# Xiuyu-Li/q-diffusion

Hardware: AMD Instinct MI355X
Metric: denoising images/sec (whole node), SD-v1.4 W4A8 512x512 50-step PLMS (higher is better)
Workload: dtype int8xint4->int32 (fp32 residual stream); 1 GPU; sd UNet eval batch 16 per GPU, 51 evals per image batch, W4A8 sm_abit=16 split, hip-graph=on, cross-attention K/V of the run's context prepared once per image batch (2.93 ms, charged as /51 per step); images_per_gpu=8, global_batch=8, context_prepared=True, parallelism=batch-sharded x1, quant-state broadcast 0 B

## Files before the change

### include/qdiff_hip.h

```cpp
#ifndef QDIFF_HIP_H
#define QDIFF_HIP_H

#include <stdint.h>

#ifdef __cplusplus
extern "C" {
#endif

#define QD_ABI_VERSION 20

enum { QD_F32 = 0, QD_F16 = 1, QD_BF16 = 2 };
enum { QD_EPI_LINEAR = 0, QD_EPI_GEGLU_I8 = 1, QD_EPI_HEADS_I8 = 2, QD_EPI_HEADS_T_I8 = 3, QD_EPI_GEGLU_H16 = 4  };

int         qd_abi_version(void);
const char* qd_last_error(void);
int         qd_device_ok(void);

int qd_box_probe(int kind, int blocks, int iters, long long* ticks, int* sink, void* stream);

int qd_make_qparams(const float* delta, const float* zero_point, float* out4, void* stream);

int qd_quantize_act(const void* x, int x_dtype, int64_t B, int64_t C, int64_t S,
                    int64_t sb, int64_t sc, int64_t ss,
                    int c0, int clen, int clen_pad,
// ... 32 lines not shown
    int32_t        out_dtype;
    int32_t        nseg;
    int32_t        w_tiled;
    int32_t        epilogue;
    qd_conv_seg    seg[2];
    const float*   oq_params;
    int32_t        oq_min, oq_max, oq_off, _pad2;
    void*          splitk_ws;
    int64_t        splitk_ws_bytes;
    int32_t        hd_H, hd_d, hd_T, hd_Tpad, hd_dpad;
    float          oq_prescale;
    int32_t*       hd_sum;
    float*         gn_part;
    int64_t        gn_ld;
    int32_t        upsample2x;
    int32_t        _pad3;
} qd_conv_desc;

int qd_conv2d_i8(const qd_conv_desc* d, void* stream);

void qd_conv_config(int kgroups);

int qd_conv2d_i8_group(const qd_conv_desc* const* descs, int n, void* stream);

int64_t qd_conv2d_i8_splitk_ws_bytes(const qd_conv_desc* d);

int qd_pack_weights_t4(const float* w, const float* alpha, const float* delta, const float* zp,
                       int Cout, int Cin_total, int taps, int c0, int clen, int clen_pad, int n_levels,
                       uint8_t* wt, int kstep0, int ntiles, int32_t* wsum, void* stream);

int qd_pack_weights_t8(const float* w, const float* alpha, const float* delta, const float* zp,
                       int Cout, int Cin_total, int taps, int c0, int clen, int clen_pad, int n_levels,
                       uint8_t* wt, int kstep0, int ntiles, int32_t* wsum, void* stream);

int qd_conv2d_i8_acc(const qd_conv_desc* d, int32_t* iout, void* stream);

// ... 112 lines not shown
```

### q-diffusion_amd/csrc/common.h

```cpp
#pragma once
#include <hip/hip_runtime.h>
#include <hip/hip_fp16.h>
#include <hip/hip_bf16.h>
#include <stdint.h>
#include <type_traits>
#include "../../include/qdiff_hip.h"

typedef int   v4i  __attribute__((ext_vector_type(4)));
typedef int   v16i __attribute__((ext_vector_type(16)));
typedef float v4f  __attribute__((ext_vector_type(4)));

void qd_set_error(const char* fmt, ...);

#define QD_REQUIRE(cond, ...)                 \
    do {                                      \
        if (!(cond)) {                        \
            qd_set_error(__VA_ARGS__);        \
            return 1;                         \
        }                                     \
    } while (0)

#define QD_LAUNCH_CHECK(name)                                                       \
    do {                                                                            \
        hipError_t e__ = hipGetLastError();                                         \
// ... 75 lines not shown
template <typename T>
__device__ __forceinline__ void qd_ld4(const T* p, bool vec, float (&v)[4]) {
    if (vec) {
        if constexpr (sizeof(T) == 4) {
            const float4 f = *reinterpret_cast<const float4*>(p);
            v[0] = f.x; v[1] = f.y; v[2] = f.z; v[3] = f.w;
        } else {
            const uint2 u = *reinterpret_cast<const uint2*>(p);
            const __half2 a = *reinterpret_cast<const __half2*>(&u.x), b = *reinterpret_cast<const __half2*>(&u.y);
            v[0] = __low2float(a); v[1] = __high2float(a); v[2] = __low2float(b); v[3] = __high2float(b);
        }
    } else {
#pragma unroll
        for (int j = 0; j < 4; ++j) v[j] = qd_ld(p + j);
    }
}

__device__ __forceinline__ float qd_erff(float a) {
    const float t = __builtin_fabsf(a), s = a * a;
    float r = __builtin_fmaf(-1.72853470e-5f, t, 3.83197126e-4f);
    const float u = __builtin_fmaf(-3.88396438e-3f, t, 2.42546219e-2f);
    r = __builtin_fmaf(r, s, u);
    r = __builtin_fmaf(r, t, -1.06777877e-1f);
    r = __builtin_fmaf(r, t, -6.34846687e-1f);
    r = __builtin_fmaf(r, t, -1.28717512e-1f);
    r = __builtin_fmaf(r, t, -t);
    const float big = __builtin_copysignf(1.0f - __builtin_amdgcn_exp2f(r * 1.4426950408889634f), a);
    float q = -5.96761703e-4f;
    q = __builtin_fmaf(q, s, 4.99119423e-3f);
    q = __builtin_fmaf(q, s, -2.67681349e-2f);
// ... 110 lines not shown
```

### q-diffusion_amd/csrc/igemm_dma.hip

```cpp
#include "common.h"
#include <type_traits>

typedef __attribute__((address_space(3))) void* qd_lds_ptr;

namespace {

__device__ __attribute__((aligned(16))) const int qd_zero16[4] = {0, 0, 0, 0};

struct SegD {
    int c0, clen, kstep0, nsteps_tap;
    const float*  scale;
    const int*    zc;
    const int*    zw;
    const int*    zfill;
    const int8_t* fill16;
};

struct ConvD {
    const int8_t*  x;
    const uint8_t* wt;
    void*          out;
    int32_t*       iout;
    const float*   bias;
    const float*   rowbias;
// ... 1122 lines not shown
        vals[j] = code;
    }
    unsigned w0 = 0, w1 = 0;
#pragma unroll
    for (int b = 0; b < 4; ++b) {
        w0 |= (unsigned)((vals[b] & 15) | ((vals[4 + b] & 15) << 4)) << (8 * b);
        w1 |= (unsigned)((vals[8 + b] & 15) | ((vals[12 + b] & 15) << 4)) << (8 * b);
    }
    const long kstep = kstep0 + (long)t * nsteps_tap + cs;
    uint2 pk = {w0, w1};
    *reinterpret_cast<uint2*>(wt + (kstep * ntiles + jt) * 1024 + (kh4 * 32 + nn) * 8) = pk;
    if (wsum && sum != 0) atomicAdd(&wsum[n], sum);
}

template <typename TO>
__global__ __launch_bounds__(256) void splitk_finalize_kernel(const int32_t* __restrict__ part, int nsplit, long MN, int Cout, int HoWo,
                                                              const float* __restrict__ scale, const int* __restrict__ zc,
                                                              const int* __restrict__ zw, const int* __restrict__ zfill,
                                                              const float* __restrict__ bias, const float* __restrict__ rowbias, long ldrb,
                                                              const TO* __restrict__ residual, long ldr, TO* __restrict__ out, long ldo) {
    const long e = (long)blockIdx.x * 256 + threadIdx.x;
    if (e >= MN) return;
    const long m = e / Cout;
    const int  n = (int)(e - m * Cout);
    int I = 0;
    for (int s = 0; s < nsplit; ++s) I += part[(long)s * MN + e];
    const int kz = zfill ? zfill[1] : 0;
    I = I - (zc ? zc[n] : 0) + (zw ? zw[n] : 0) * kz;
    float v = __builtin_fmaf((float)I, scale[n], bias ? bias[n] : 0.f);
    if (rowbias) v += rowbias[(m / HoWo) * ldrb + n];
    if constexpr (std::is_same<TO, float>::value) {
        if (residual) v += residual[m * ldr + n];
        out[m * ldo + n] = v;
    } else {
        if (residual) v += __half2float(residual[m * ldr + n]);
        out[m * ldo + n] = __float2half(v);
    }
}

__global__ __launch_bounds__(256) void pack_t8_kernel(const float* __restrict__ w, const float* __restrict__ alpha,
                                                      const float* __restrict__ delta, const float* __restrict__ zp,
                                                      int Cout, int Cin_total, int taps, int c0, int clen,
                                                      int n_levels, uint8_t* __restrict__ wt, int kstep0, int ntiles,
                                                      int nsteps_tap, int32_t* __restrict__ wsum) {
    long gid = (long)blockIdx.x * 256 + threadIdx.x;
    const long total = (long)taps * nsteps_tap * ntiles * 128;
    if (gid >= total) return;
    const int nn = (int)(gid & 31);
    const int kh4 = (int)((gid >> 5) & 3);
    long rest = gid >> 7;
    const int jt = (int)(rest % ntiles);
// ... 80 lines not shown
        QD_CASE(false, O_F32) QD_CASE(false, O_F16)
    } else {
        QD_CASE(false, O_F32)
        QD_CASE(false, O_F16)
        if constexpr (MT == 1 && WM == 4) { QD_CASE(false, O_I32) QD_CASE(true, O_F32) QD_CASE(true, O_F16) QD_CASE(false, O_PART) }
        if constexpr ((WB == 4 && WM == 4) || (WB == 8 && MT == 1 && NT == 4)) { QD_CASE(false, O_HROWS) QD_CASE(false, O_HTR) }
        if constexpr (NT == 4 && WB == 4 && WM == 4) { QD_CASE(false, O_GEGLU) }
    }
#undef QD_CASE
    qd_set_error("qd_conv2d_%s: unsupported variant split=%d out=%d tile %dx%d", WB >= 16 ? "bf16" : "i8", (int)split, out, BM, BN);
    return 1;
}

int nt_for(int N) { return N % 160 == 0 ? 5 : (N % 224 == 0 ? 7 : (N > 64 ? 4 : 2)); }

int choose_splitk(const qd_conv_desc* d, int* it_per) {
    *it_per = 0;
    if (d->nseg != 1 || d->epilogue != QD_EPI_LINEAR) return 1;
    const long M = (long)d->B * d->Ho * d->Wo;
    const int  N = d->Cout, bn = 32 * (d->wbits == 8 ? (N > 64 ? 4 : 2) : nt_for(N));
    const long blocks0 = ((M + 127) / 128) * ((N + bn - 1) / bn);
    const int  total = d->kh * d->kw * ((d->seg[0].clen + 63) / 64);
    if (blocks0 > 256) return 1;
    const long mn = M * N;
    const int min_steps = mn <= (1L << 18) ? 2 : (mn <= (3L << 19) ? 4 : 16);
    static const long target = getenv("QD_SPLITK_TARGET") ? atol(getenv("QD_SPLITK_TARGET")) : 256;
    long S = target / blocks0;
    if (S > total / min_steps) S = total / min_steps;
    if (S > 32) S = 32;
    if (S < 2) return 1;
    *it_per = (int)((total + S - 1) / S);
    return (total + *it_per - 1) / *it_per;
}

int run(const qd_conv_desc* d, int32_t* iout, void* stream) {
    QD_REQUIRE(d != nullptr, "qd_conv2d_i8: null descriptor");
    QD_REQUIRE(d->x && d->w && (d->out || iout), "qd_conv2d_i8: null tensor pointer");
// ... 52 lines not shown
        QD_REQUIRE(d->hd_Tpad % 32 == 0 && d->hd_Tpad >= d->hd_T && d->hd_dpad >= d->hd_d, "qd_conv2d_i8: heads epilogue: bad padded dims");
        QD_REQUIRE(qd_aligned(d->out, 16) && (d->epilogue != QD_EPI_HEADS_T_I8 || d->hd_sum), "qd_conv2d_i8: heads epilogue: out unaligned or hd_sum missing");
        QD_REQUIRE(!d->rowbias && (!d->residual || (d->epilogue == QD_EPI_HEADS_I8 && d->ldr % 4 == 0 && qd_aligned(d->residual, 4 * esz))),
                   "qd_conv2d_i8: heads epilogue takes no rowbias; a residual (fp32 or fp16 as out_dtype says, 4-element aligned rows) only with QD_EPI_HEADS_I8");
        k.res_f16 = d->out_dtype == QD_F16 ? 1 : 0;
        k.vec = (d->epilogue == QD_EPI_HEADS_I8 && d->hd_d % 8 == 0 && d->hd_dpad % 8 == 0 && d->Cout % 8 == 0 && qd_aligned(d->out, 8) &&
                 (!d->residual || (d->ldr % 8 == 0 && qd_aligned(d->residual, 16)))) ? 2 : 1;
        k.oq = d->oq_params; k.oqmin = (float)d->oq_min; k.oqmax = (float)d->oq_max; k.oqoff = d->oq_off;
        k.hdH = d->hd_H; k.hdd = d->hd_d; k.hdT = d->hd_T; k.hdTpad = d->hd_Tpad; k.hddpad = d->hd_dpad;
        k.oqpre = d->oq_prescale; k.hdsum = d->hd_sum;
        QD_REQUIRE(d->Cout < 65536, "qd_conv2d_i8: heads epilogue: Cout must be < 65536");
        k.hdrcp = (unsigned)((0x100000000ULL + (unsigned)d->hd_d - 1) / (unsigned)d->hd_d);
    }
    if (d->gn_part) {
        QD_REQUIRE(!iout && !heads && !geglu, "qd_conv2d_i8: gn_part needs the plain fp32 / fp16 epilogue");
        QD_REQUIRE((d->Ho * d->Wo) % 128 == 0, "qd_conv2d_i8: gn_part needs Ho*Wo %% 128 == 0 (a 128-row chunk stays inside one sample)");
        k.gnpart = d->gn_part;
        k.gn_nchunk = d->Ho * d->Wo / 128;
        QD_REQUIRE(d->gn_ld == 0 || d->gn_ld >= d->Cout, "qd_conv2d_i8: gn_ld must be 0 or >= Cout");
        k.gn_ld = d->gn_ld ? (long)d->gn_ld : (long)d->Cout;
    }
    const bool mt2_ok = !heads || d->hd_T % 256 == 0;
    if (geglu) {
        QD_REQUIRE(!iout && d->nseg == 1 && d->oq_params && d->Cout % 64 == 0, "qd_conv2d_i8: GEGLU epilogue needs one segment, oq_params and Cout %% 64 == 0");
        QD_REQUIRE(d->oq_max - d->oq_off <= 127 && d->oq_min - d->oq_off >= -128, "qd_conv2d_i8: GEGLU output grid does not fit int8");
        QD_REQUIRE(d->ldo % 16 == 0 && qd_aligned(d->out, 16), "qd_conv2d_i8: GEGLU output rows must be 16-byte aligned");
        k.oq = d->oq_params; k.oqmin = (float)d->oq_min; k.oqmax = (float)d->oq_max; k.oqoff = d->oq_off;
    }
    QD_REQUIRE(!(iout && split), "qd_conv2d_i8_acc: single segment only");
    hipStream_t st = reinterpret_cast<hipStream_t>(stream);
    const int N = d->Cout;
    const long M = k.M;
    int rc;
    auto blocks = [&](int bm, int bn) { return ((M + bm - 1) / bm) * ((N + bn - 1) / bn); };
    int it_per = 0;
    const int nsplit = (iout || !d->splitk_ws || d->gn_part) ? 1 : choose_splitk(d, &it_per);
    if (nsplit >= 2 && d->splitk_ws_bytes >= (int64_t)nsplit * M * N * 4) {
        QD_REQUIRE(qd_aligned(d->splitk_ws, 16), "qd_conv2d_i8: splitk_ws must be 16-byte aligned");
        k.iout = reinterpret_cast<int32_t*>(d->splitk_ws);
        k.it_per = it_per;
        k.vec = N % 4 == 0;
        if (w8) rc = N > 64 ? dispatch<1, 4, 4, 1, 8>(k, false, O_PART, st, nsplit) : dispatch<1, 2, 4, 1, 8>(k, false, O_PART, st, nsplit);
        else switch (nt_for(N)) {
            case 5:  rc = dispatch<1, 5, 4, 1>(k, false, O_PART, st, nsplit); break;
            case 7:  rc = dispatch<1, 7, 4, 1>(k, false, O_PART, st, nsplit); break;
            case 4:  rc = dispatch<1, 4, 4, 1>(k, false, O_PART, st, nsplit); break;
            default: rc = dispatch<1, 2, 4, 1>(k, false, O_PART, st, nsplit); break;
        }
        if (rc || g_capture) return rc;
        const SegD& sg = k.seg[0];
        const long MN = M * N;
        dim3 grid((unsigned)((MN + 255) / 256)), block(256);
        if (d->out_dtype == QD_F16)
            hipLaunchKernelGGL(splitk_finalize_kernel<__half>, grid, block, 0, st, k.iout, nsplit, MN, N, d->Ho * d->Wo, sg.scale, sg.zc, sg.zw,
                               sg.zfill, k.bias, k.rowbias, k.ldrb, (const __half*)k.residual, k.ldr, (__half*)k.out, k.ldo);
        else
            hipLaunchKernelGGL(splitk_finalize_kernel<float>, grid, block, 0, st, k.iout, nsplit, MN, N, d->Ho * d->Wo, sg.scale, sg.zc, sg.zw,
                               sg.zfill, k.bias, k.rowbias, k.ldrb, (const float*)k.residual, k.ldr, (float*)k.out, k.ldo);
        QD_LAUNCH_CHECK("qd_conv2d_i8 (split-K)");
        return 0;
    }
    static const int wide_mink = getenv("QD_WIDE_MINK") ? atoi(getenv("QD_WIDE_MINK")) : 1280;
    static const int wide_minblk = getenv("QD_WIDE_MINBLK") ? atoi(getenv("QD_WIDE_MINBLK")) : 200;
    const long Ktot = (long)k.taps * d->seg[0].clen;
    const bool linear_out = out == O_F32 || out == O_F16;
    auto want_mt2 = [&](int bn) {
        if (split || !mt2_ok || out == O_I32) return false;
        if (g_capture) return false;
// ... 177 lines not shown
        if (ok) {
            QD_LAUNCH_CHECK("qd_conv2d_i8_group");
            return 0;
        }
    }
    for (int i = 0; i < n; ++i) {
        const int rc = run(descs[i], nullptr, stream);
        if (rc) return rc;
    }
    return 0;
}

extern "C" void qd_conv_config(int kgroups) {
    if (kgroups >= 0) kgroups_knob() = kgroups ? 1 : 0;
}
extern "C" int qd_conv2d_i8_group(const qd_conv_desc* const* descs, int n, void* stream) { return run_group(descs, n, stream); }
extern "C" int qd_conv2d_i8(const qd_conv_desc* d, void* stream) { return run(d, nullptr, stream); }
extern "C" int qd_conv2d_i8_acc(const qd_conv_desc* d, int32_t* iout, void* stream) {
    if (!iout) { qd_set_error("qd_conv2d_i8_acc: null iout"); return 1; }
    return run(d, iout, stream);
}

extern "C" int qd_pack_weights_t4(const float* w, const float* alpha, const float* delta, const float* zp, int Cout,
                                  int Cin_total, int taps, int c0, int clen, int clen_pad, int n_levels, uint8_t* wt,
                                  int kstep0, int ntiles, int32_t* wsum, void* stream) {
    QD_REQUIRE(w && delta && zp && wt, "qd_pack_weights_t4: null pointer");
    QD_REQUIRE(Cout > 0 && taps > 0 && clen > 0 && c0 >= 0 && c0 + clen <= Cin_total, "qd_pack_weights_t4: bad shape");
    QD_REQUIRE(clen_pad % 16 == 0 && clen_pad >= clen, "qd_pack_weights_t4: clen_pad must be a multiple of 16");
    QD_REQUIRE(n_levels >= 2 && n_levels <= 16, "qd_pack_weights_t4: n_levels %d does not fit a nibble", n_levels);
    QD_REQUIRE(ntiles == (Cout + 31) / 32 && qd_aligned(wt, 16), "qd_pack_weights_t4: bad tile layout");
// ... 584 lines not shown
```

### q-diffusion_amd/csrc/norm_quant.hip

```cpp
#include "common.h"

namespace {

static inline __host__ __device__ int gn_rows(long S) { return S > 256 ? 32 : 8; }

template <typename T>
__global__ __launch_bounds__(256) void gn_partial_kernel(const T* __restrict__ x, long S, int C, long ldx,
                                                         float* __restrict__ part, int nchunk, int vec) {
    const int chunk = blockIdx.x;
    const long b = blockIdx.y;
    const int rows = gn_rows(S);
    const long r0 = (long)chunk * rows;
    const long r1 = (r0 + rows < S) ? r0 + rows : S;
    for (int c4 = threadIdx.x; c4 < C / 4; c4 += 256) {
        float s[4] = {0, 0, 0, 0}, q[4] = {0, 0, 0, 0};
        const T* p = x + (b * S + r0) * ldx + c4 * 4;
#pragma unroll 4
        for (long r = r0; r < r1; ++r, p += ldx) {
            float v[4];
            qd_ld4(p, vec != 0, v);
#pragma unroll
            for (int j = 0; j < 4; ++j) {
                s[j] += v[j];
                q[j] += v[j] * v[j];
            }
        }
        float* dst = part + (((b * nchunk + chunk) * (long)C) + c4 * 4) * 2;
        *reinterpret_cast<float4*>(dst)     = make_float4(s[0], q[0], s[1], q[1]);
        *reinterpret_cast<float4*>(dst + 4) = make_float4(s[2], q[2], s[3], q[3]);
    }
}

__global__ __launch_bounds__(256) void gn_partial_h8_kernel(const __half* __restrict__ x, long S, int C, long ldx,
                                                            float* __restrict__ part, int nchunk) {
    const int chunk = blockIdx.x;
    const long b = blockIdx.y;
    const int rows = gn_rows(S);
    const long r0 = (long)chunk * rows;
    const long r1 = (r0 + rows < S) ? r0 + rows : S;
    for (int c8 = threadIdx.x; c8 < C / 8; c8 += 256) {
        float s[8] = {0, 0, 0, 0, 0, 0, 0, 0}, q[8] = {0, 0, 0, 0, 0, 0, 0, 0};
        const __half* p = x + (b * S + r0) * ldx + c8 * 8;
#pragma unroll 4
        for (long r = r0; r < r1; ++r, p += ldx) {
            float v[8];
            qd_ld8h(p, v);
#pragma unroll
            for (int j = 0; j < 8; ++j) {
                s[j] += v[j];
                q[j] += v[j] * v[j];
            }
        }
        float* dst = part + (((b * nchunk + chunk) * (long)C) + c8 * 8) * 2;
#pragma unroll
        for (int j = 0; j < 4; ++j) *reinterpret_cast<float4*>(dst + 4 * j) = make_float4(s[2 * j], q[2 * j], s[2 * j + 1], q[2 * j + 1]);
    }
}

template <int NT>
__global__ __launch_bounds__(NT) void gn_finalize_kernel(const float* __restrict__ part, int nchunk, long ldp, long S, int C,
                                                         int groups, float eps, const float* __restrict__ gamma,
                                                         const float* __restrict__ beta, float* __restrict__ ab) {
    static_assert(NT == 64 || NT == 256, "one wave, or four whose results are added in wave order");
    const int g = blockIdx.x;
    const long b = blockIdx.y;
    const int cpg = C / groups;
// ... 1026 lines not shown
```

### q-diffusion_amd/qdiff/engine.py

```python
import math

import os

import torch

from . import hip
from .hip import Grid, pad16, pad32

SIMULATE = False


class simulation:

    def __enter__(self):
        global SIMULATE
        self.prev, SIMULATE = SIMULATE, True
        return self

    def __exit__(self, *exc):
        global SIMULATE
        SIMULATE = self.prev
        return False


# ... 283 lines not shown

    def __init__(self, slot, i):
        self.slot, self.i = slot, i

    def rows(self, M, C, device):
        return self.slot.rows(self.i, M, C, device)

    def part(self, B, nchunk, C, device):
        return self.slot.part(self.i, B, nchunk, C, device)


def upsample_fold_ok(plan, H, W):
    return bool(plan.pack.tiled and plan.kh * plan.kw > 1 and plan.stride == 1 and H % 2 == 0 and W % 2 == 0)


def conv_forward(plan, xq, B, H, W, Ho=None, Wo=None, out=None, rowbias=None, residual=None, acc_out=None,
                 out_dtype=None, pad_tl=None, splitk=None, gn_stats=False, slot=None, upsample2x=False):
    if Ho is None:
        Ho, Wo = conv_out_hw(H, W, plan)
    M = B * Ho * Wo
    if out_dtype is None:
        out_dtype = out.dtype if out is not None else stream_dtype()
    if residual is not None and acc_out is None and residual.dtype != out_dtype:
        residual = residual.to(out_dtype)
    if out is None and acc_out is None:
        if slot is not None and out_dtype == stream_dtype():
            out = slot.rows(M, plan.Cout, xq.device)
        if out is None:
            slot = None
            out = torch.empty((M, plan.Cout), dtype=out_dtype, device=xq.device)
    else:
        slot = None
    pad = plan.pad if pad_tl is None else pad_tl
    call = hip.ConvCall(x=xq, w=plan.pack.wq, out=out, bias=plan.bias, rowbias=rowbias,
                        residual=residual, ldx=plan.ldx, ldk=plan.pack.ldk,
                        ldo=(out.stride(0) if out is not None else 0),
                        ldr=(residual.stride(0) if residual is not None else 0),
                        ld_rowbias=(rowbias.stride(0) if rowbias is not None else 0),
                        B=B, H=H, W=W, Ho=Ho, Wo=Wo, Cout=plan.Cout, kh=plan.kh, kw=plan.kw, stride=plan.stride,
                        pad_t=pad, pad_l=pad, wbits=plan.pack.wbits, w_tiled=plan.pack.tiled, segs=plan.segs,
                        splitk=splitk, upsample2x=upsample2x)
    part = None
    if (gn_stats and acc_out is None and plan.pack.tiled and out.dtype in (torch.float32, torch.float16) and (Ho * Wo) % 128 == 0
            and out.stride(1) == 1 and (splitk is False or hip.splitk_ws_bytes(call) == 0)):
        if slot is not None:
            part = slot.part(B, Ho * Wo // 128, plan.Cout, xq.device)
        if part is None:
            part = torch.empty((B, Ho * Wo // 128, plan.Cout, 2), dtype=torch.float32, device=xq.device)
        call.gn_part = part
    hip.conv2d_i8(call, acc_out=acc_out)
    if part is not None:
        out.qd_gn_part = part
    return out if acc_out is None else acc_out


def conv_forward_geglu(plan, xq, M, next_plan):
    if not plan.pack.tiled or plan.pack.wbits != 4 or plan.pack.row_perm is None or len(plan.segs) != 1 or len(next_plan.segs) != 1:
        raise hip.HipEngineError("fused GEGLU epilogue needs a tile-ordered int4 projection packed with geglu_row_perm")
    out = torch.empty((M, next_plan.ldx), dtype=torch.int8, device=xq.device)
    call = hip.ConvCall(x=xq, w=plan.pack.wq, out=out, bias=plan.bias, ldx=plan.ldx, ldk=plan.pack.ldk, ldo=next_plan.ldx,
                        B=1, H=1, W=M, Ho=1, Wo=M, Cout=plan.Cout, kh=1, kw=1, stride=1, pad_t=0, pad_l=0,
                        wbits=plan.pack.wbits, w_tiled=True, segs=plan.segs, epilogue=hip.EPI_GEGLU_I8,
                        oq_params=next_plan.qparams[0], oq_grid=next_plan.grids[0])
    hip.conv2d_i8(call)
# ... 314 lines not shown


_ws_cache = {}


def _workspace(nbytes, device):
    key = (device, torch.cuda.current_stream().cuda_stream if device.type == "cuda" else 0)
    buf = _ws_cache.get(key)
    if buf is None or buf.numel() < nbytes:
        buf = torch.empty(max(nbytes, 1 << 20), dtype=torch.uint8, device=device)
        _ws_cache[key] = buf
    return buf


def _part_view(part, B, S, C):
    if part is None or S % 128 != 0 or part.dim() != 4 or part.shape[2] != C or part.shape[0] * part.shape[1] * 128 != B * S:
        return None
    if tuple(part.shape[:2]) == (B, S // 128):
        return part
    try:
        return part.view(B, S // 128, C, 2)
    except RuntimeError:
        return None


def raw_quant_segs(plan, C):
    segs, pos = [], 0
    for sg, d, grid, qp in zip(plan.pack.segs, plan.segs, plan.grids, plan.qparams):
        if sg["clen"] % 16 or sg["c0w"] % 16 or d["c0"] % 16 or sg["c0w"] != pos:
            return None
        segs.append(dict(c0=sg["c0w"], clen=sg["clen"], oc0=d["c0"], qparams=qp, grid=grid))
        pos += sg["clen"]
    return segs if pos == C and 1 <= len(segs) <= 2 else None


def groupnorm_silu_quant(x_rows, B, S, C, gn, silu, plan=None, want_float=False, part=None, raw_plan=None, mod=None):
# ... 285 lines not shown
```

### q-diffusion_amd/qdiff/hip.py

```python
import ctypes
import os

import torch

_HERE = os.path.dirname(os.path.abspath(__file__))
LIB_PATH = os.environ.get("QDIFF_HIP_LIB") or os.path.join(os.path.dirname(_HERE), "lib", "libqdiff_hip.so")

F32, F16, BF16 = 0, 1, 2
_DT = {torch.float32: F32, torch.float16: F16}


class HipEngineError(RuntimeError):
    pass


class ConvSeg(ctypes.Structure):
    _fields_ = [("c0", ctypes.c_int32), ("clen", ctypes.c_int32), ("kofs", ctypes.c_int32), ("kstep0", ctypes.c_int32),
                ("wzp", ctypes.c_void_p), ("scale", ctypes.c_void_p), ("zc", ctypes.c_void_p), ("zw", ctypes.c_void_p), ("zfill", ctypes.c_void_p),
                ("fill16", ctypes.c_void_p)]


class ConvDesc(ctypes.Structure):
    _fields_ = [("x", ctypes.c_void_p), ("w", ctypes.c_void_p), ("out", ctypes.c_void_p),
                ("bias", ctypes.c_void_p), ("rowbias", ctypes.c_void_p), ("residual", ctypes.c_void_p),
                ("ldx", ctypes.c_int64), ("ldk", ctypes.c_int64), ("ldo", ctypes.c_int64), ("ldr", ctypes.c_int64),
                ("ld_rowbias", ctypes.c_int64),
                ("B", ctypes.c_int32), ("H", ctypes.c_int32), ("W", ctypes.c_int32), ("Ho", ctypes.c_int32),
                ("Wo", ctypes.c_int32), ("Cout", ctypes.c_int32),
                ("kh", ctypes.c_int32), ("kw", ctypes.c_int32), ("stride", ctypes.c_int32), ("pad_t", ctypes.c_int32),
                ("pad_l", ctypes.c_int32),
                ("wbits", ctypes.c_int32), ("out_dtype", ctypes.c_int32), ("nseg", ctypes.c_int32),
                ("w_tiled", ctypes.c_int32), ("epilogue", ctypes.c_int32),
                ("seg", ConvSeg * 2),
                ("oq_params", ctypes.c_void_p), ("oq_min", ctypes.c_int32), ("oq_max", ctypes.c_int32),
                ("oq_off", ctypes.c_int32), ("_pad2", ctypes.c_int32),
                ("splitk_ws", ctypes.c_void_p), ("splitk_ws_bytes", ctypes.c_int64),
                ("hd_H", ctypes.c_int32), ("hd_d", ctypes.c_int32), ("hd_T", ctypes.c_int32), ("hd_Tpad", ctypes.c_int32),
                ("hd_dpad", ctypes.c_int32), ("oq_prescale", ctypes.c_float), ("hd_sum", ctypes.c_void_p),
                ("gn_part", ctypes.c_void_p), ("gn_ld", ctypes.c_int64), ("upsample2x", ctypes.c_int32), ("_pad3", ctypes.c_int32)]


class RawSeg(ctypes.Structure):
    _fields_ = [("c0", ctypes.c_int32), ("clen", ctypes.c_int32), ("oc0", ctypes.c_int32),
                ("qmin", ctypes.c_int32), ("qmax", ctypes.c_int32), ("off", ctypes.c_int32), ("qparams", ctypes.c_void_p)]


class RawQuant(ctypes.Structure):
    _fields_ = [("out", ctypes.c_void_p), ("ldo", ctypes.c_int64), ("nseg", ctypes.c_int32), ("_pad", ctypes.c_int32),
                ("seg", RawSeg * 2)]


EPI_LINEAR, EPI_GEGLU_I8, EPI_HEADS_I8, EPI_HEADS_T_I8 = 0, 1, 2, 3
EPI_GEGLU_H16 = 4


EXPORTS = ["qd_abi_version", "qd_last_error", "qd_device_ok", "qd_box_probe", "qd_make_qparams", "qd_quantize_act", "qd_pack_weights", "qd_pack_weights_t4",
           "qd_pack_weights_t8",
           "qd_conv2d_i8", "qd_conv_config", "qd_conv2d_i8_group", "qd_conv2d_i8_splitk_ws_bytes",
           "qd_conv2d_i8_acc", "qd_groupnorm_ws_bytes", "qd_groupnorm_silu_quant", "qd_groupnorm_mod_silu_quant", "qd_layernorm_quant",
           "qd_geglu_quant", "qd_quantize_heads", "qd_attn_i8", "qd_attn_keyterm", "qd_attn_uses_keyterm", "qd_attn_config", "qd_attn_ws_bytes", "qd_bmm_qk_i8", "qd_bmm_pv_i8", "qd_temb_mlp",
           "qd_fakequant_blocks", "qd_fakequant_fwd", "qd_fakequant_bwd",
           "qd_conv2d_bf16", "qd_pack_weights_bf16_bytes", "qd_pack_weights_bf16", "qd_groupnorm_silu_bf16",
           "qd_pack_weights_h16", "qd_groupnorm_silu_h16", "qd_conv2d_wq_h16", "qd_rows_to_h16",
           "qd_conv2d_wq_h16_splitk_ws_bytes", "qd_wq_h16_config",
           "qd_attn_h16", "qd_layernorm_h16", "qd_geglu_h16", "qd_groupnorm_h16", "qd_groupnorm_mod_h16", "qd_groupnorm_resample_h16"]

_lib = None


def load():
    global _lib
    if _lib is not None:
        return _lib
    if not os.path.exists(LIB_PATH):
        raise HipEngineError(f"{LIB_PATH} not found: build it with `python q-diffusion_amd/build.py` "
                             "(or __graft_entry__.build()); the quantised path has no fallback")
    lib = ctypes.CDLL(LIB_PATH)
    lib.qd_last_error.restype = ctypes.c_char_p
    lib.qd_groupnorm_ws_bytes.restype = ctypes.c_int64
    lib.qd_groupnorm_ws_bytes.argtypes = [ctypes.c_int64] * 3
    i64, i32, vp, f32 = ctypes.c_int64, ctypes.c_int, ctypes.c_void_p, ctypes.c_float
    lib.qd_make_qparams.argtypes = [vp, vp, vp, vp]
    lib.qd_quantize_act.argtypes = [vp, i32, i64, i64, i64, i64, i64, i64, i32, i32, i32, vp, i32, i32, i32, vp, i64, i32, vp]
    lib.qd_pack_weights.argtypes = [vp, vp, vp, vp, i32, i32, i32, i32, i32, i32, i32, i32, vp, i64, i32, vp, vp, vp]
    lib.qd_pack_weights_t4.argtypes = [vp, vp, vp, vp, i32, i32, i32, i32, i32, i32, i32, vp, i32, i32, vp, vp]
    lib.qd_pack_weights_t8.argtypes = [vp, vp, vp, vp, i32, i32, i32, i32, i32, i32, i32, vp, i32, i32, vp, vp]
    lib.qd_conv2d_i8.argtypes = [ctypes.POINTER(ConvDesc), vp]
    lib.qd_conv_config.argtypes = [i32]
    lib.qd_conv_config.restype = None
    lib.qd_conv2d_i8_group.argtypes = [ctypes.POINTER(ctypes.POINTER(ConvDesc)), i32, vp]
    lib.qd_conv2d_i8_acc.argtypes = [ctypes.POINTER(ConvDesc), vp, vp]
    lib.qd_conv2d_i8_splitk_ws_bytes.argtypes = [ctypes.POINTER(ConvDesc)]
    lib.qd_conv2d_i8_splitk_ws_bytes.restype = ctypes.c_int64
    lib.qd_groupnorm_silu_quant.argtypes = [vp, i32, i64, i64, i32, i64, i32, f32, vp, vp, i32, vp, i32, i32, i32, vp,
                                            i64, vp, i64, vp, vp, i32, i64, ctypes.POINTER(RawQuant), vp]
    lib.qd_groupnorm_mod_silu_quant.argtypes = [vp, i32, i64, i64, i32, i64, i32, f32, vp, vp, i32, vp, i32, i32, i32, vp,
                                                i64, vp, i64, vp, vp, i32, i64, vp, i64, vp]
    lib.qd_layernorm_quant.argtypes = [vp, i32, i64, i32, i64, f32, vp, vp, i32, ctypes.POINTER(vp),
                                       ctypes.POINTER(i32), ctypes.POINTER(i32), ctypes.POINTER(i32),
                                       ctypes.POINTER(vp), i64, vp]
    lib.qd_geglu_quant.argtypes = [vp, i32, i64, i32, i64, vp, i32, i32, i32, vp, i64, vp]
    lib.qd_quantize_heads.argtypes = [vp, i32, i32, i32, i32, i32, i64, i64, i64, i64, f32, vp, i32, i32, i32, i32,
                                      vp, vp, i32, i32, vp]
    lib.qd_attn_i8.argtypes = [vp, vp, vp, vp, vp, vp, i32, i32, i32, i32, i32, i32, i32, i32, vp, i32, i32, i32, i32, vp,
# ... 25 lines not shown
    lib.qd_attn_h16.argtypes = [vp, vp, vp, i32, i32, i32, i32, i32, i32] + [i64] * 12 + [f32, i32, vp, i32, i64, vp]
    lib.qd_layernorm_h16.argtypes = [vp, i32, i64, i32, i64, f32, vp, vp, vp, i32, i64, vp]
    lib.qd_geglu_h16.argtypes = [vp, i32, i64, i32, i64, vp, i32, i64, vp]
    lib.qd_groupnorm_h16.argtypes = [vp, i32, i64, i64, i32, i64, i32, f32, vp, vp, i32, vp, i32, i64, vp, vp]
    lib.qd_groupnorm_mod_h16.argtypes = [vp, i32, i64, i64, i32, i64, i32, f32, vp, vp, vp, i64, i32, vp, i32, i64, vp, vp]
    lib.qd_groupnorm_resample_h16.argtypes = [vp, i32, i64, i32, i32, i32, i64, i32, f32, vp, vp, i32, i32, vp, i32, i64, vp, vp]
    lib.qd_box_probe.argtypes = [i32, i32, i32, vp, vp, vp]
    lib.qd_attn_ws_bytes.argtypes = [i32, i32, i32, i32]
    lib.qd_attn_ws_bytes.restype = ctypes.c_int64
    if lib.qd_abi_version() != 20:
        raise HipEngineError("libqdiff_hip.so ABI version mismatch")
    _lib = lib
    return lib


def available():
    try:
        return bool(load().qd_device_ok())
    except (HipEngineError, OSError):
        return False


def _check(rc, what):
    if rc != 0:
        raise HipEngineError(f"{what} failed ({rc}): {load().qd_last_error().decode()}")


def _ptr(t, name="tensor"):
    if t is None:
        return None
# ... 61 lines not shown
def pack_weights_t4(w, alpha, delta, zp, Cout, Cin_total, taps, c0, clen, n_levels, wt, kstep0, ntiles, wsum):
    _check(load().qd_pack_weights_t4(_ptr(w), _ptr(alpha), _ptr(delta), _ptr(zp), Cout, Cin_total, taps, c0, clen,
                                     pad16(clen), n_levels, _ptr(wt), kstep0, ntiles, _ptr(wsum), _stream()),
           "qd_pack_weights_t4")


def pack_weights_t8(w, alpha, delta, zp, Cout, Cin_total, taps, c0, clen, n_levels, wt, kstep0, ntiles, wsum):
    _check(load().qd_pack_weights_t8(_ptr(w), _ptr(alpha), _ptr(delta), _ptr(zp), Cout, Cin_total, taps, c0, clen,
                                     pad16(clen), n_levels, _ptr(wt), kstep0, ntiles, _ptr(wsum), _stream()),
           "qd_pack_weights_t8")


class ConvCall:
    __slots__ = ("x", "w", "out", "bias", "rowbias", "residual", "ldx", "ldk", "ldo", "ldr", "ld_rowbias",
                 "B", "H", "W", "Ho", "Wo", "Cout", "kh", "kw", "stride", "pad_t", "pad_l", "wbits", "w_tiled", "segs",
                 "epilogue", "oq_params", "oq_grid", "splitk", "heads", "gn_part", "upsample2x", "_keep")

    def __init__(self, **kw):
        for k in self.__slots__:
            setattr(self, k, kw.get(k))


_SPLITK_WS = {}


def _splitk_scratch(device, nbytes):
    bufs = _SPLITK_WS.setdefault((device, _stream()), [])
    if not bufs or bufs[-1].numel() < nbytes:
        bufs.append(torch.empty(max(nbytes, 64 << 20), dtype=torch.uint8, device=device))
    return bufs[-1]

# ... 3 lines not shown


def conv2d_i8(c, acc_out=None):
    d = _conv_desc(c)
    if acc_out is None:
        if c.w_tiled and c.splitk is not False:
            need = int(load().qd_conv2d_i8_splitk_ws_bytes(ctypes.byref(d)))
            if need:
                ws = _splitk_scratch(c.x.device, need)
                d.splitk_ws, d.splitk_ws_bytes = ws.data_ptr(), ws.numel()
        _check(load().qd_conv2d_i8(ctypes.byref(d), _stream()), "qd_conv2d_i8")
    else:
        _check(load().qd_conv2d_i8_acc(ctypes.byref(d), _ptr(acc_out), _stream()), "qd_conv2d_i8_acc")


def conv_config(kgroups=-1):
    load().qd_conv_config(int(kgroups))


def conv2d_i8_group(calls):
    descs = [_conv_desc(c) for c in calls]
    arr = (ctypes.POINTER(ConvDesc) * len(descs))(*[ctypes.pointer(d) for d in descs])
    _check(load().qd_conv2d_i8_group(arr, len(descs), _stream()), "qd_conv2d_i8_group")


def _conv_desc(c):
    d = ConvDesc()
    d.x, d.w = _ptr(c.x, "x"), _ptr(c.w, "w")
    d.out = _ptr(c.out, "out")
    d.bias, d.rowbias, d.residual = _ptr(c.bias, "bias"), _ptr(c.rowbias, "rowbias"), _ptr(c.residual, "residual")
    d.ldx, d.ldk, d.ldo = c.ldx, c.ldk, c.ldo or 0
    d.ldr, d.ld_rowbias = c.ldr or 0, c.ld_rowbias or 0
# ... 7 lines not shown
        d.oq_params = _ptr(c.oq_params, "oq_params")
        d.oq_min, d.oq_max, d.oq_off = c.oq_grid.qmin, c.oq_grid.qmax, c.oq_grid.off
        d.out_dtype = _dtype(c.residual) if c.residual is not None else F32
        if d.epilogue in (EPI_HEADS_I8, EPI_HEADS_T_I8):
            hd = c.heads
            d.hd_H, d.hd_d, d.hd_T, d.hd_Tpad, d.hd_dpad = hd["H"], hd["d"], hd["T"], hd["Tpad"], hd["dpad"]
            d.oq_prescale = float(hd["prescale"])
            d.hd_sum = _ptr(hd.get("sum"), "hd_sum")
    elif d.epilogue == EPI_GEGLU_H16:
        d.out_dtype = _H16[c.out.dtype]
    else:
        d.out_dtype = _dtype(c.out) if c.out is not None else F32
    d.gn_part = _ptr(c.gn_part, "gn_part")
    if c.gn_part is not None:
        d.gn_ld = part_ld(c.gn_part)
    d.upsample2x = 1 if c.upsample2x else 0
    d.nseg = len(c.segs)
    for i, s in enumerate(c.segs):
        g = d.seg[i]
        g.c0, g.clen, g.kofs, g.kstep0 = s["c0"], s["clen"], s["kofs"], s.get("kstep0", 0)
        g.wzp, g.fill16 = _ptr(s.get("wzp"), "wzp"), _ptr(s.get("fill16"), "fill16")
        g.scale, g.zc, g.zw, g.zfill = _ptr(s["scale"], "scale"), _ptr(s.get("zc")), _ptr(s.get("zw")), _ptr(s.get("zfill"))
    return d



def pad8(n):
    return (n + 7) // 8 * 8


# ... 369 lines not shown
```

Baseline: 8.720 images/s.

## Fuse GroupNorm partial statistics into the split-K finalize kernel

Split-K conv launches used to fall back to a separate GroupNorm partial-statistics pass because the fused gn_part path required an unsplit launch. A new finalize kernel sums the split-K partials, applies the epilogue, stores the output, and also reduces per-chunk sum and sum-of-squares through LDS in the gn_rows chunk layout. Python chooses the chunk count from the split decision, and _part_view now accepts that layout. The change also adds a split-K override knob, which is off by default. The trade-off is lower parallelism in the finalize step, since each thread handles a 64-column tile over several rows.

```diff
diff --git a/include/qdiff_hip.h b/include/qdiff_hip.h
--- a/include/qdiff_hip.h
+++ b/include/qdiff_hip.h
@@ -70,12 +70,14 @@
     float*         gn_part;
     int64_t        gn_ld;
     int32_t        upsample2x;
-    int32_t        _pad3;
+    int32_t        gn_split;
 } qd_conv_desc;
 
 int qd_conv2d_i8(const qd_conv_desc* d, void* stream);
 
 void qd_conv_config(int kgroups);
+
+void qd_conv_splitk_config(int nsplit);
 
 int qd_conv2d_i8_group(const qd_conv_desc* const* descs, int n, void* stream);
 
diff --git a/q-diffusion_amd/csrc/common.h b/q-diffusion_amd/csrc/common.h
--- a/q-diffusion_amd/csrc/common.h
+++ b/q-diffusion_amd/csrc/common.h
@@ -113,6 +113,12 @@
 #pragma unroll
         for (int j = 0; j < 4; ++j) v[j] = qd_ld(p + j);
     }
+}
+
+static inline __host__ __device__ int qd_gn_rows(long S) { return S > 256 ? 32 : 8; }
+__device__ __forceinline__ void qd_gn_acc(float& s, float& q, float v) {
+    s += v;
+    q = __builtin_fmaf(v, v, q);
 }
 
 __device__ __forceinline__ float qd_erff(float a) {
diff --git a/q-diffusion_amd/csrc/igemm_dma.hip b/q-diffusion_amd/csrc/igemm_dma.hip
--- a/q-diffusion_amd/csrc/igemm_dma.hip
+++ b/q-diffusion_amd/csrc/igemm_dma.hip
@@ -1160,6 +1160,25 @@
 }
 
 template <typename TO>
+__device__ __forceinline__ float splitk_value(const int32_t* __restrict__ part, int nsplit, long MN, long e, long m, int n, int HoWo,
+                                              const float* __restrict__ scale, const int* __restrict__ zc, const int* __restrict__ zw,
+                                              const int* __restrict__ zfill, const float* __restrict__ bias,
+                                              const float* __restrict__ rowbias, long ldrb, const TO* __restrict__ residual, long ldr) {
+    int I = 0;
+    for (int s = 0; s < nsplit; ++s) I += part[(long)s * MN + e];
+    const int kz = zfill ? zfill[1] : 0;
+    I = I - (zc ? zc[n] : 0) + (zw ? zw[n] : 0) * kz;
+    float v = __builtin_fmaf((float)I, scale[n], bias ? bias[n] : 0.f);
+    if (rowbias) v += rowbias[(m / HoWo) * ldrb + n];
+    if constexpr (std::is_same<TO, float>::value) {
+        if (residual) v += residual[m * ldr + n];
+    } else {
+        if (residual) v += __half2float(residual[m * ldr + n]);
+    }
+    return v;
+}
+
+template <typename TO>
 __global__ __launch_bounds__(256) void splitk_finalize_kernel(const int32_t* __restrict__ part, int nsplit, long MN, int Cout, int HoWo,
                                                               const float* __restrict__ scale, const int* __restrict__ zc,
                                                               const int* __restrict__ zw, const int* __restrict__ zfill,
@@ -1169,18 +1188,47 @@
     if (e >= MN) return;
     const long m = e / Cout;
     const int  n = (int)(e - m * Cout);
-    int I = 0;
-    for (int s = 0; s < nsplit; ++s) I += part[(long)s * MN + e];
-    const int kz = zfill ? zfill[1] : 0;
-    I = I - (zc ? zc[n] : 0) + (zw ? zw[n] : 0) * kz;
-    float v = __builtin_fmaf((float)I, scale[n], bias ? bias[n] : 0.f);
-    if (rowbias) v += rowbias[(m / HoWo) * ldrb + n];
-    if constexpr (std::is_same<TO, float>::value) {
-        if (residual) v += residual[m * ldr + n];
-        out[m * ldo + n] = v;
-    } else {
-        if (residual) v += __half2float(residual[m * ldr + n]);
-        out[m * ldo + n] = __float2half(v);
+    const float v = splitk_value<TO>(part, nsplit, MN, e, m, n, HoWo, scale, zc, zw, zfill, bias, rowbias, ldrb, residual, ldr);
+    if constexpr (std::is_same<TO, float>::value) out[m * ldo + n] = v;
+    else out[m * ldo + n] = __float2half(v);
+}
+
+template <typename TO>
+__global__ __launch_bounds__(256) void splitk_finalize_gn_kernel(const int32_t* __restrict__ part, int nsplit, long MN, int Cout, int HoWo,
+                                                                 const float* __restrict__ scale, const int* __restrict__ zc,
+                                                                 const int* __restrict__ zw, const int* __restrict__ zfill,
+                                                                 const float* __restrict__ bias, const float* __restrict__ rowbias, long ldrb,
+                                                                 const TO* __restrict__ residual, long ldr, TO* __restrict__ out, long ldo,
+                                                                 float* __restrict__ gnpart, int nchunk, long gn_ld) {
+    __shared__ float vals[32][64];
+    const int tx = threadIdx.x & 63, ry = threadIdx.x >> 6;
+    const int n = blockIdx.x * 64 + tx;
+    const long b = blockIdx.y / nchunk;
+    const int chunk = blockIdx.y - (int)b * nchunk;
+    const int rows = qd_gn_rows(HoWo);
+    const int r0 = chunk * rows;
+    const int r1 = (r0 + rows < HoWo) ? r0 + rows : HoWo;
+    if (n < Cout) {
+#pragma unroll 2
+        for (int r = r0 + ry; r < r1; r += 4) {
+            const long m = b * HoWo + r;
+            const long e = m * Cout + n;
+            float v = splitk_value<TO>(part, nsplit, MN, e, m, n, HoWo, scale, zc, zw, zfill, bias, rowbias, ldrb, residual, ldr);
+            if constexpr (std::is_same<TO, float>::value) {
+                out[m * ldo + n] = v;
+            } else {
+                const __half h = __float2half(v);
+                out[m * ldo + n] = h;
+                v = __half2float(h);
+            }
+            vals[r - r0][tx] = v;
+        }
+    }
+    __syncthreads();
+    if (ry == 0 && n < Cout) {
+        float s = 0.f, q = 0.f;
+        for (int r = 0; r < r1 - r0; ++r) qd_gn_acc(s, q, vals[r][tx]);
+        *reinterpret_cast<float2*>(gnpart + ((b * nchunk + chunk) * gn_ld + n) * 2) = make_float2(s, q);
     }
 }
 
@@ -1291,6 +1339,11 @@
 
 int nt_for(int N) { return N % 160 == 0 ? 5 : (N % 224 == 0 ? 7 : (N > 64 ? 4 : 2)); }
 
+static int& splitk_knob() {
+    static int v = 0;
+    return v;
+}
+
 int choose_splitk(const qd_conv_desc* d, int* it_per) {
     *it_per = 0;
     if (d->nseg != 1 || d->epilogue != QD_EPI_LINEAR) return 1;
@@ -1298,6 +1351,12 @@
     const int  N = d->Cout, bn = 32 * (d->wbits == 8 ? (N > 64 ? 4 : 2) : nt_for(N));
     const long blocks0 = ((M + 127) / 128) * ((N + bn - 1) / bn);
     const int  total = d->kh * d->kw * ((d->seg[0].clen + 63) / 64);
+    if (splitk_knob() >= 2) {
+        const int want = splitk_knob() < total ? splitk_knob() : total;
+        if (want < 2) return 1;
+        *it_per = (total + want - 1) / want;
+        return (total + *it_per - 1) / *it_per;
+    }
     if (blocks0 > 256) return 1;
     const long mn = M * N;
     const int min_steps = mn <= (1L << 18) ? 2 : (mn <= (3L << 19) ? 4 : 16);
@@ -1380,7 +1439,9 @@
     }
     if (d->gn_part) {
         QD_REQUIRE(!iout && !heads && !geglu, "qd_conv2d_i8: gn_part needs the plain fp32 / fp16 epilogue");
-        QD_REQUIRE((d->Ho * d->Wo) % 128 == 0, "qd_conv2d_i8: gn_part needs Ho*Wo %% 128 == 0 (a 128-row chunk stays inside one sample)");
+        QD_REQUIRE(d->gn_split || (d->Ho * d->Wo) % 128 == 0, "qd_conv2d_i8: gn_part needs Ho*Wo %% 128 == 0 (a 128-row chunk stays inside one sample)");
+        QD_REQUIRE(!d->gn_split || (d->splitk_ws && !split), "qd_conv2d_i8: gn_split needs a split-K launch (splitk_ws, one segment)");
+        QD_REQUIRE(!d->gn_split || (long)d->B * ((d->Ho * d->Wo + 7) / 8) <= 65535, "qd_conv2d_i8: gn_split: too many statistics chunks for one launch");
         k.gnpart = d->gn_part;
         k.gn_nchunk = d->Ho * d->Wo / 128;
         QD_REQUIRE(d->gn_ld == 0 || d->gn_ld >= d->Cout, "qd_conv2d_i8: gn_ld must be 0 or >= Cout");
@@ -1400,7 +1461,9 @@
     int rc;
     auto blocks = [&](int bm, int bn) { return ((M + bm - 1) / bm) * ((N + bn - 1) / bn); };
     int it_per = 0;
-    const int nsplit = (iout || !d->splitk_ws || d->gn_part) ? 1 : choose_splitk(d, &it_per);
+    const int nsplit = (iout || !d->splitk_ws || (d->gn_part && !d->gn_split)) ? 1 : choose_splitk(d, &it_per);
+    QD_REQUIRE(!(d->gn_part && d->gn_split) || (nsplit >= 2 && d->splitk_ws_bytes >= (int64_t)nsplit * M * N * 4),
+               "qd_conv2d_i8: gn_split, but this launch does not split K (qd_conv2d_i8_splitk_ws_bytes says which do)");
     if (nsplit >= 2 && d->splitk_ws_bytes >= (int64_t)nsplit * M * N * 4) {
         QD_REQUIRE(qd_aligned(d->splitk_ws, 16), "qd_conv2d_i8: splitk_ws must be 16-byte aligned");
         k.iout = reinterpret_cast<int32_t*>(d->splitk_ws);
@@ -1417,7 +1480,16 @@
         const SegD& sg = k.seg[0];
         const long MN = M * N;
         dim3 grid((unsigned)((MN + 255) / 256)), block(256);
-        if (d->out_dtype == QD_F16)
+        if (d->gn_part) {
+            const int HoWo = d->Ho * d->Wo, nchunk = (HoWo + qd_gn_rows(HoWo) - 1) / qd_gn_rows(HoWo);
+            const dim3 ggrid((unsigned)((N + 63) / 64), (unsigned)((long)d->B * nchunk));
+            if (d->out_dtype == QD_F16)
+                hipLaunchKernelGGL(splitk_finalize_gn_kernel<__half>, ggrid, block, 0, st, k.iout, nsplit, MN, N, HoWo, sg.scale, sg.zc, sg.zw,
+                                   sg.zfill, k.bias, k.rowbias, k.ldrb, (const __half*)k.residual, k.ldr, (__half*)k.out, k.ldo, k.gnpart, nchunk, k.gn_ld);
+            else
+                hipLaunchKernelGGL(splitk_finalize_gn_kernel<float>, ggrid, block, 0, st, k.iout, nsplit, MN, N, HoWo, sg.scale, sg.zc, sg.zw,
+                                   sg.zfill, k.bias, k.rowbias, k.ldrb, (const float*)k.residual, k.ldr, (float*)k.out, k.ldo, k.gnpart, nchunk, k.gn_ld);
+        } else if (d->out_dtype == QD_F16)
             hipLaunchKernelGGL(splitk_finalize_kernel<__half>, grid, block, 0, st, k.iout, nsplit, MN, N, d->Ho * d->Wo, sg.scale, sg.zc, sg.zw,
                                sg.zfill, k.bias, k.rowbias, k.ldrb, (const __half*)k.residual, k.ldr, (__half*)k.out, k.ldo);
         else
@@ -1625,6 +1697,9 @@
 extern "C" void qd_conv_config(int kgroups) {
     if (kgroups >= 0) kgroups_knob() = kgroups ? 1 : 0;
 }
+extern "C" void qd_conv_splitk_config(int nsplit) {
+    if (nsplit >= 0) splitk_knob() = nsplit >= 2 ? (nsplit > 32 ? 32 : nsplit) : 0;
+}
 extern "C" int qd_conv2d_i8_group(const qd_conv_desc* const* descs, int n, void* stream) { return run_group(descs, n, stream); }
 extern "C" int qd_conv2d_i8(const qd_conv_desc* d, void* stream) { return run(d, nullptr, stream); }
 extern "C" int qd_conv2d_i8_acc(const qd_conv_desc* d, int32_t* iout, void* stream) {
diff --git a/q-diffusion_amd/csrc/norm_quant.hip b/q-diffusion_amd/csrc/norm_quant.hip
--- a/q-diffusion_amd/csrc/norm_quant.hip
+++ b/q-diffusion_amd/csrc/norm_quant.hip
@@ -2,7 +2,7 @@
 
 namespace {
 
-static inline __host__ __device__ int gn_rows(long S) { return S > 256 ? 32 : 8; }
+static inline __host__ __device__ int gn_rows(long S) { return qd_gn_rows(S); }
 
 template <typename T>
 __global__ __launch_bounds__(256) void gn_partial_kernel(const T* __restrict__ x, long S, int C, long ldx,
@@ -20,10 +20,7 @@
             float v[4];
             qd_ld4(p, vec != 0, v);
 #pragma unroll
-            for (int j = 0; j < 4; ++j) {
-                s[j] += v[j];
-                q[j] += v[j] * v[j];
-            }
+            for (int j = 0; j < 4; ++j) qd_gn_acc(s[j], q[j], v[j]);
         }
         float* dst = part + (((b * nchunk + chunk) * (long)C) + c4 * 4) * 2;
         *reinterpret_cast<float4*>(dst)     = make_float4(s[0], q[0], s[1], q[1]);
@@ -46,10 +43,7 @@
             float v[8];
             qd_ld8h(p, v);
 #pragma unroll
-            for (int j = 0; j < 8; ++j) {
-                s[j] += v[j];
-                q[j] += v[j] * v[j];
-            }
+            for (int j = 0; j < 8; ++j) qd_gn_acc(s[j], q[j], v[j]);
         }
         float* dst = part + (((b * nchunk + chunk) * (long)C) + c8 * 8) * 2;
 #pragma unroll
diff --git a/q-diffusion_amd/qdiff/engine.py b/q-diffusion_amd/qdiff/engine.py
--- a/q-diffusion_amd/qdiff/engine.py
+++ b/q-diffusion_amd/qdiff/engine.py
@@ -321,6 +321,15 @@
     return bool(plan.pack.tiled and plan.kh * plan.kw > 1 and plan.stride == 1 and H % 2 == 0 and W % 2 == 0)
 
 
+SPLITK_GN_STATS = True
+SPLITK_GN_LAUNCHES = [0]
+
+
+def gn_chunks(S):
+    rows = 32 if S > 256 else 8
+    return (S + rows - 1) // rows
+
+
 def conv_forward(plan, xq, B, H, W, Ho=None, Wo=None, out=None, rowbias=None, residual=None, acc_out=None,
                  out_dtype=None, pad_tl=None, splitk=None, gn_stats=False, slot=None, upsample2x=False):
     if Ho is None:
@@ -348,13 +357,21 @@
                         pad_t=pad, pad_l=pad, wbits=plan.pack.wbits, w_tiled=plan.pack.tiled, segs=plan.segs,
                         splitk=splitk, upsample2x=upsample2x)
     part = None
-    if (gn_stats and acc_out is None and plan.pack.tiled and out.dtype in (torch.float32, torch.float16) and (Ho * Wo) % 128 == 0
-            and out.stride(1) == 1 and (splitk is False or hip.splitk_ws_bytes(call) == 0)):
-        if slot is not None:
-            part = slot.part(B, Ho * Wo // 128, plan.Cout, xq.device)
-        if part is None:
-            part = torch.empty((B, Ho * Wo // 128, plan.Cout, 2), dtype=torch.float32, device=xq.device)
-        call.gn_part = part
+    if (gn_stats and acc_out is None and plan.pack.tiled and out.dtype in (torch.float32, torch.float16) and out.stride(1) == 1):
+        S = Ho * Wo
+        split = splitk is not False and hip.splitk_ws_bytes(call) > 0
+        if not split:
+            nchunk = S // 128 if S % 128 == 0 else 0
+        else:
+            nchunk = gn_chunks(S) if SPLITK_GN_STATS and hip.splitk_gn_ok() else 0
+        if nchunk:
+            if slot is not None:
+                part = slot.part(B, nchunk, plan.Cout, xq.device)
+            if part is None:
+                part = torch.empty((B, nchunk, plan.Cout, 2), dtype=torch.float32, device=xq.device)
+            call.gn_part, call.gn_split = part, split
+            if split:
+                SPLITK_GN_LAUNCHES[0] += 1
     hip.conv2d_i8(call, acc_out=acc_out)
     if part is not None:
         out.qd_gn_part = part
@@ -699,12 +716,20 @@
 
 
 def _part_view(part, B, S, C):
-    if part is None or S % 128 != 0 or part.dim() != 4 or part.shape[2] != C or part.shape[0] * part.shape[1] * 128 != B * S:
+    if part is None or part.dim() != 4 or part.shape[2] != C:
         return None
-    if tuple(part.shape[:2]) == (B, S // 128):
+    total = part.shape[0] * part.shape[1]
+    rows = 32 if S > 256 else 8
+    if S % 128 == 0 and total * 128 == B * S:
+        nchunk = S // 128
+    elif total == B * gn_chunks(S) and (part.shape[0] == B or S % rows == 0):
+        nchunk = gn_chunks(S)
+    else:
+        return None
+    if tuple(part.shape[:2]) == (B, nchunk):
         return part
     try:
-        return part.view(B, S // 128, C, 2)
+        return part.view(B, nchunk, C, 2)
     except RuntimeError:
         return None
 
diff --git a/q-diffusion_amd/qdiff/hip.py b/q-diffusion_amd/qdiff/hip.py
--- a/q-diffusion_amd/qdiff/hip.py
+++ b/q-diffusion_amd/qdiff/hip.py
@@ -37,7 +37,7 @@
                 ("splitk_ws", ctypes.c_void_p), ("splitk_ws_bytes", ctypes.c_int64),
                 ("hd_H", ctypes.c_int32), ("hd_d", ctypes.c_int32), ("hd_T", ctypes.c_int32), ("hd_Tpad", ctypes.c_int32),
                 ("hd_dpad", ctypes.c_int32), ("oq_prescale", ctypes.c_float), ("hd_sum", ctypes.c_void_p),
-                ("gn_part", ctypes.c_void_p), ("gn_ld", ctypes.c_int64), ("upsample2x", ctypes.c_int32), ("_pad3", ctypes.c_int32)]
+                ("gn_part", ctypes.c_void_p), ("gn_ld", ctypes.c_int64), ("upsample2x", ctypes.c_int32), ("gn_split", ctypes.c_int32)]
 
 
 class RawSeg(ctypes.Structure):
@@ -56,7 +56,7 @@
 
 EXPORTS = ["qd_abi_version", "qd_last_error", "qd_device_ok", "qd_box_probe", "qd_make_qparams", "qd_quantize_act", "qd_pack_weights", "qd_pack_weights_t4",
            "qd_pack_weights_t8",
-           "qd_conv2d_i8", "qd_conv_config", "qd_conv2d_i8_group", "qd_conv2d_i8_splitk_ws_bytes",
+           "qd_conv2d_i8", "qd_conv_config", "qd_conv_splitk_config", "qd_conv2d_i8_group", "qd_conv2d_i8_splitk_ws_bytes",
            "qd_conv2d_i8_acc", "qd_groupnorm_ws_bytes", "qd_groupnorm_silu_quant", "qd_groupnorm_mod_silu_quant", "qd_layernorm_quant",
            "qd_geglu_quant", "qd_quantize_heads", "qd_attn_i8", "qd_attn_keyterm", "qd_attn_uses_keyterm", "qd_attn_config", "qd_attn_ws_bytes", "qd_bmm_qk_i8", "qd_bmm_pv_i8", "qd_temb_mlp",
            "qd_fakequant_blocks", "qd_fakequant_fwd", "qd_fakequant_bwd",
@@ -66,6 +66,7 @@
            "qd_attn_h16", "qd_layernorm_h16", "qd_geglu_h16", "qd_groupnorm_h16", "qd_groupnorm_mod_h16", "qd_groupnorm_resample_h16"]
 
 _lib = None
+_splitk_gn = False
 
 
 def load():
@@ -88,6 +89,11 @@
     lib.qd_conv2d_i8.argtypes = [ctypes.POINTER(ConvDesc), vp]
     lib.qd_conv_config.argtypes = [i32]
     lib.qd_conv_config.restype = None
+    global _splitk_gn
+    _splitk_gn = hasattr(lib, "qd_conv_splitk_config")
+    if _splitk_gn:
+        lib.qd_conv_splitk_config.argtypes = [i32]
+        lib.qd_conv_splitk_config.restype = None
     lib.qd_conv2d_i8_group.argtypes = [ctypes.POINTER(ctypes.POINTER(ConvDesc)), i32, vp]
     lib.qd_conv2d_i8_acc.argtypes = [ctypes.POINTER(ConvDesc), vp, vp]
     lib.qd_conv2d_i8_splitk_ws_bytes.argtypes = [ctypes.POINTER(ConvDesc)]
@@ -143,6 +149,11 @@
     return lib
 
 
+def splitk_gn_ok():
+    load()
+    return _splitk_gn
+
+
 def available():
     try:
         return bool(load().qd_device_ok())
@@ -234,7 +245,7 @@
 class ConvCall:
     __slots__ = ("x", "w", "out", "bias", "rowbias", "residual", "ldx", "ldk", "ldo", "ldr", "ld_rowbias",
                  "B", "H", "W", "Ho", "Wo", "Cout", "kh", "kw", "stride", "pad_t", "pad_l", "wbits", "w_tiled", "segs",
-                 "epilogue", "oq_params", "oq_grid", "splitk", "heads", "gn_part", "upsample2x", "_keep")
+                 "epilogue", "oq_params", "oq_grid", "splitk", "heads", "gn_part", "gn_split", "upsample2x", "_keep")
 
     def __init__(self, **kw):
         for k in self.__slots__:
@@ -268,8 +279,12 @@
         _check(load().qd_conv2d_i8_acc(ctypes.byref(d), _ptr(acc_out), _stream()), "qd_conv2d_i8_acc")
 
 
-def conv_config(kgroups=-1):
+def conv_config(kgroups=-1, splitk=-1):
     load().qd_conv_config(int(kgroups))
+    if splitk != -1:
+        if not splitk_gn_ok():
+            raise HipEngineError("conv_config(splitk=...): this libqdiff_hip.so has no qd_conv_splitk_config")
+        load().qd_conv_splitk_config(int(splitk))
 
 
 def conv2d_i8_group(calls):
@@ -307,6 +322,7 @@
     d.gn_part = _ptr(c.gn_part, "gn_part")
     if c.gn_part is not None:
         d.gn_ld = part_ld(c.gn_part)
+        d.gn_split = 1 if c.gn_split else 0
     d.upsample2x = 1 if c.upsample2x else 0
     d.nseg = len(c.segs)
     for i, s in enumerate(c.segs):
```

Result: no change. 8.767 images/s (median of 3 runs) (+0.5%).
